# ponimatkin/freepose

Hardware: AMD Instinct MI355X
Metric: proposals/sec (ViT-L feat + top-k + 576-pose render-compare) (higher is better)
Workload: dtype bf16

## Files before the change

freepose_amd/_lib.py:

```python
from __future__ import annotations

import ctypes as C
import os
from pathlib import Path

_HERE = Path(__file__).resolve().parent
LIB_PATH = _HERE / "lib" / "libfreepose_hip.so"
LAB_LIB_PATH = _HERE / "lib" / "libfreepose_hip_lab.so"

_lib = None
_use_lab = False


def use_lab():
    global _use_lab
    if _lib is not None and not _use_lab:
        raise RuntimeError("use_lab() after the product library was loaded")
    _use_lab = True


def is_lab() -> bool:
    return _use_lab

c_void_p, c_int, c_float, c_double, c_size_t, c_char_p = C.c_void_p, C.c_int, C.c_float, C.c_double, C.c_size_t, C.c_char_p
# ... 4 lines not shown
    _fields_ = [("dim", c_int), ("depth", c_int), ("heads", c_int), ("mlp_dim", c_int), ("patch", c_int),
                ("n_reg", c_int), ("pos_grid", c_int), ("ln_eps", c_float)]


SIGNATURES = {
    "fp_last_error": (c_char_p, []),
    "fp_version": (c_int, []),
    "fp_ctx_create": (c_int, [c_int, P(c_void_p)]),
    "fp_ctx_destroy": (c_int, [c_void_p]),
    "fp_ctx_set_option": (c_int, [c_void_p, c_char_p, c_int]),
    "fp_ctx_workspace_bytes": (c_size_t, [c_void_p]),
    "fp_vit_create": (c_int, [c_void_p, P(VitArch), P(c_void_p)]),
    "fp_vit_destroy": (c_int, [c_void_p]),
    "fp_vit_set_weight": (c_int, [c_void_p, c_char_p, c_void_p, c_size_t, c_void_p]),
    "fp_vit_forward": (c_int, [c_void_p, c_void_p, c_int, c_int, c_int, c_int, c_int, c_void_p, c_void_p]),
    "fp_vit_flops": (c_double, [c_void_p, c_int, c_int, c_int, c_int]),
    "fp_ffa": (c_int, [c_void_p, c_void_p, c_void_p, c_int, c_int, c_int, c_int, c_int, c_int, c_void_p, c_void_p, c_void_p]),
    "fp_bank_prepare": (c_int, [c_void_p, c_void_p, c_int, c_int, c_void_p, c_void_p]),
    "fp_bank_topk": (c_int, [c_void_p, c_void_p, c_int, c_int, c_void_p, c_int, c_int, c_int, c_void_p, c_void_p, c_void_p]),
    "fp_topk_merge": (c_int, [c_void_p, c_void_p, c_void_p, c_int, c_int, c_int, c_void_p, c_void_p, c_void_p]),
    "fp_rerank_views": (c_int, [c_void_p, c_void_p, c_void_p, c_void_p, c_void_p, c_int, c_int, c_int, c_int, c_void_p, c_void_p]),
    "fp_l2_normalize": (c_int, [c_void_p, c_void_p, c_int, c_int, c_void_p, c_void_p]),
    "fp_template_score": (c_int, [c_void_p, c_void_p, c_void_p, c_void_p, c_int, c_int, c_int, c_void_p, c_void_p]),
    "fp_template_score_normed": (c_int, [c_void_p, c_void_p, c_void_p, c_void_p, c_int, c_int, c_int, c_void_p, c_void_p]),
    "fp_crop_resize_pad": (c_int, [c_void_p, c_void_p, c_int, c_int, c_int, c_int, c_int, c_void_p, c_int, c_float,
                                   c_int, c_void_p, c_int, c_void_p, c_int, c_void_p]),
    "fp_roi_align": (c_int, [c_void_p, c_void_p, c_int, c_int, c_int, c_int, c_void_p, c_int, c_int, c_int, c_int, c_float,
                             c_void_p, c_void_p]),
    "fp_generate_rotations": (c_int, [c_int, c_void_p]),
    "fp_geodesic_select": (c_int, [c_void_p, c_void_p, c_int, c_void_p, c_double, c_void_p, P(c_int), c_void_p]),
    "fp_mesh_upload": (c_int, [c_void_p, c_void_p, c_int, c_void_p, c_int, c_void_p, P(c_void_p)]),
    "fp_mesh_upload_textured": (c_int, [c_void_p, c_void_p, c_int, c_void_p, c_int, c_void_p, c_void_p, c_int, c_int, c_void_p,
                                        P(c_void_p)]),
    "fp_mesh_set_ambient": (c_int, [c_void_p, c_float]),
    "fp_mesh_set_shading": (c_int, [c_void_p, c_int]),
    "fp_mesh_set_filter": (c_int, [c_void_p, c_int]),
    "fp_mesh_set_cull": (c_int, [c_void_p, c_int]),
    "fp_project_vertices": (c_int, [c_void_p, c_void_p, c_void_p, c_int, c_float, c_float, c_float, c_float, c_float, c_void_p,
                                    c_void_p, c_void_p]),
    "fp_mesh_destroy": (c_int, [c_void_p]),
    "fp_rasterize": (c_int, [c_void_p, c_void_p, c_void_p, c_int, c_float, c_float, c_float, c_float, c_float, c_int,
# ... 81 lines not shown
```

freepose_amd/csrc/capi.hip:

```cpp
#include <stdarg.h>
#include <stdio.h>
#include <string.h>
#include <stdlib.h>

#include <cmath>

#include "../../include/freepose_hip.h"
#include "internal.h"

static thread_local char g_err[512] = "";
void fp_set_error(const char* fmt, ...) {
    va_list ap;
    va_start(ap, fmt);
    vsnprintf(g_err, sizeof(g_err), fmt, ap);
    va_end(ap);
}
extern "C" const char* fp_last_error(void) { return g_err; }
extern "C" int fp_version(void) { return 100; }

#ifdef FP_LAB
static int g_opts[FP_OPT_COUNT] = {-1, -1, -1, -1, -1, -1, -1, -1, -1, -1, -1, -1};
int fp_opt_get(int key, int dflt) { return (key >= 0 && key < FP_OPT_COUNT && g_opts[key] >= 0) ? g_opts[key] : dflt; }
extern "C" int fp_lab_set_option(const char* name, int value) {
    FP_REQUIRE(name, "lab_set_option: null name");
// ... 294 lines not shown
        if (v->ev_used == v->ev_pool.size()) {
            fp_vit::EvPair p{};
            if (hipEventCreate(&p.a) != hipSuccess || hipEventCreate(&p.b) != hipSuccess) return;
            v->ev_pool.push_back(p);
        }
        slot = v->ev_used++;
        v->ev_pool[slot].cls = cls;
        (void)hipEventRecord(v->ev_pool[slot].a, s);
    }
    ~ProfScope() {
        if (slot != (size_t)-1) (void)hipEventRecord(v->ev_pool[slot].b, s);
    }
};
}

extern "C" int fp_vit_forward(fp_vit* v, const void* d_images, int B, int H, int W, int layer, int feature_type,
                              void* d_out, void* stream) {
    FP_REQUIRE(v && d_images && d_out, "vit_forward: null argument");
    const fp_vit_arch& a = v->a;
    hipStream_t s = (hipStream_t)stream;
    FP_REQUIRE(B > 0 && H % a.patch == 0 && W % a.patch == 0, "vit_forward: B=%d H=%d W=%d (patch %d)", B, H, W, a.patch);
    FP_REQUIRE(feature_type >= 0 && feature_type <= 3, "vit_forward: feature_type %d", feature_type);
    FP_REQUIRE(v->cls && v->pos && v->pe_b && v->normw && v->normb && (a.n_reg == 0 || v->reg),
               "vit_forward: embedding / final-norm weights not set");
    const int L = (layer >= 1 && layer <= a.depth) ? layer : a.depth;
    for (int i = 0; i < L; ++i) {
        const VitBlockW& w = v->blk[i];
        FP_REQUIRE(w.n1w && w.n1b && w.qkvw && w.qkvb && w.projw && w.projb && w.n2w && w.n2b && w.fc1w && w.fc1b &&
                       w.fc2w && w.fc2b, "vit_forward: weights of block %d not set", i);
    }
    const int D = a.dim, gh = H / a.patch, gw = W / a.patch, P = gh * gw;
    const int n_tok = P + 1 + a.n_reg;
    const int npad = cdiv(n_tok, 16) * 16;
    const size_t M = (size_t)B * npad;
    FP_REQUIRE(M * (size_t)a.mlp_dim * 2 < 0xffffffffull, "vit_forward: batch too large for 32-bit tile offsets (B=%d)", B);

    bf16_t *A0, *X, *Y, *QK, *Vt, *AO, *H1;
    int rc;
    const int nosplit = v->ctx->opt_row_split == 0;
    const bool lnf = v->ctx->opt_ln_fused != 0 && D % 64 == 0;
    uint4* stat = nullptr;
    float2* part = nullptr;
    float* rstd = nullptr;
    if (lnf) {
        if (v->fold_ev && s != v->fold_stream) FP_HIP(hipStreamWaitEvent(s, v->fold_ev, 0));
        if (v->folded_upto < L) {
            if (v->refold) {
                FP_HIP(hipDeviceSynchronize());
                v->refold = false;
            }
            if ((rc = vit_fold(v, v->folded_upto, L, s))) return rc;
            if (!v->fold_ev) FP_HIP(hipEventCreateWithFlags(&v->fold_ev, hipEventDisableTiming));
            FP_HIP(hipEventRecord(v->fold_ev, s));
            v->fold_stream = s;
            v->folded_upto = L;
        }
        if ((rc = v->ctx->get("vit.ln_stat", M * sizeof(uint4), (void**)&stat))) return rc;
        if ((rc = v->ctx->get("vit.ln_rstd", M * sizeof(float), (void**)&rstd))) return rc;
        if ((rc = v->ctx->get("vit.ln_part", M * (size_t)(D / 64) * sizeof(float2), (void**)&part))) return rc;
    }
    if ((rc = v->ctx->get("vit.im2col", (size_t)B * P * v->KP * 2, (void**)&A0))) return rc;
    if ((rc = v->ctx->get("vit.x", M * D * 2, (void**)&X))) return rc;
    if ((rc = v->ctx->get("vit.y", M * D * 2, (void**)&Y))) return rc;
    if ((rc = v->ctx->get("vit.qk", M * 2 * D * 2, (void**)&QK))) return rc;
    if ((rc = v->ctx->get("vit.vt", M * D * 2 + 256, (void**)&Vt))) return rc;
    if ((rc = v->ctx->get("vit.ao", M * D * 2, (void**)&AO))) return rc;
    if ((rc = v->ctx->get("vit.h1", M * (size_t)a.mlp_dim * 2, (void**)&H1))) return rc;

    const bf16_t* pos_patch;
    if ((rc = vit_pos(v, gh, gw, s, &pos_patch))) return rc;

    {
        ProfScope ps(v, s, &v->ms_other);
        if ((rc = fp_im2col_norm((const bf16_t*)d_images, A0, B, H, W, a.patch, v->KP, s))) return rc;
        if ((rc = fp_token_init(X, v->cls, v->pos, v->reg, a.n_reg, B, n_tok, npad, D, s))) return rc;
    }
    {
        ProfScope ps(v, s, &v->ms_gemm);
        FpGemmArgs g{}; g.no_split = nosplit; if ((rc = v->ctx->sk_scratch(g, s))) return rc;
        g.X = A0; g.ldx = v->KP; g.W = v->pe_w; g.ldw = v->KP; g.C = X; g.ldc = D; g.bias = v->pe_b;
        g.M = B * P; g.N = D; g.K = v->KP; g.pos = pos_patch; g.P = P; g.npad = npad; g.tok_off = 1 + a.n_reg;
        if ((rc = fp_gemm_bf16(g, FP_EPI_PATCH, s))) return rc;
        if (v->prof) { v->gemm_flops += 2.0 * g.M * (3.0 * a.patch * a.patch) * D; v->gemm_launches += 1; }
    }
    const int Mi = (int)M;
    const double Malg = (double)B * n_tok;
    for (int i = 0; i < L; ++i) {
        const VitBlockW& w = v->blk[i];
        const fp_vit::VitFold& f = v->fold[i];
// ... 51 lines not shown
    }
    {
        ProfScope ps(v, s, &v->ms_other);
        int rows_per_b, off;
        if (feature_type == 0) { rows_per_b = 1; off = 0; }
        else if (feature_type == 1) { rows_per_b = a.n_reg; off = 1; }
        else { rows_per_b = P; off = 1 + a.n_reg; }
        if (rows_per_b > 0)
            if ((rc = fp_layernorm(X, (bf16_t*)d_out, v->normw, v->normb, B * rows_per_b, D, a.ln_eps, rows_per_b, npad,
                                   off, s, feature_type == 3)))
                return rc;
    }
    return FP_OK;
}

extern "C" int fp_vit_profile(fp_vit* v, int enable) {
    FP_REQUIRE(v, "vit_profile: null");
    v->prof = enable != 0;
    v->ev_used = 0;
    v->ms_gemm = v->ms_attn = v->ms_other = 0;
    v->gemm_flops = 0;
    v->gemm_launches = 0;
    return FP_OK;
}
extern "C" int fp_vit_profile_read(fp_vit* v, float* g, float* at, float* o, double* fl) {
    FP_REQUIRE(v, "vit_profile_read: null");
    float acc[3] = {0.f, 0.f, 0.f};
    for (size_t i = 0; i < v->ev_used; ++i) {
        FP_HIP(hipEventSynchronize(v->ev_pool[i].b));
        float ms = 0.f;
// ... 250 lines not shown
```

freepose_amd/csrc/internal.h:

```cpp
#pragma once
#include <algorithm>
#include <map>
#include <string>
#include <vector>

#include "common.h"
#include "gemm_bf16.h"

struct fp_ctx {
    int device = 0;
    struct Buf { void* p = nullptr; size_t bytes = 0; };
    std::map<std::string, Buf> bufs;
    int get(const char* name, size_t bytes, void** out);
    void* comm = nullptr;
    int comm_rank = 0, comm_size = 1;
    int opt_ln_fused = -1;
    int opt_raster_tiled = -1;
    int opt_comm_timeout_s = -1;
    int opt_row_split = -1;
    int opt_stream_k = -1;
    float* sk_ws = nullptr;
    int* sk_cnt = nullptr;
    static constexpr size_t SK_WS_BYTES = (size_t)64 << 20;
    static constexpr int SK_CNT_N = 16384;
    int sk_scratch(FpGemmArgs& g, hipStream_t s);
    int* ffa_arrive = nullptr;
    size_t total() const;
    void release();
};

constexpr float FP_ATTN_QSCALE = 1.4426950408889634f / 8.0f;
int fp_attention_fwd(const bf16_t* QK, int ldqk, const bf16_t* Vt, bf16_t* O, int ldo, int B, int H, int n_tok,
                     int npad, bool q_prescaled, hipStream_t stream);
int fp_im2col_norm(const bf16_t* img, bf16_t* A, int B, int H, int W, int ps, int KP, hipStream_t s);
int fp_token_init(bf16_t* X, const bf16_t* cls, const bf16_t* pos0, const bf16_t* reg, int nreg, int B, int n_tok,
                  int npad, int D, hipStream_t s);
int fp_layernorm(const bf16_t* X, bf16_t* Y, const bf16_t* gamma, const bf16_t* beta, int rows, int D, float eps,
                 int rows_per_b, int in_stride_b, int in_off, hipStream_t s, int l2_normalize = 0);
int fp_posembed_aa(const bf16_t* src, bf16_t* dst, int G, int gh, int gw, int D, hipStream_t s);
int fp_ffa_pool(const bf16_t* feats, const uint8_t* mask, bf16_t* out, float* out_f32, int B, int P, int D, int gh,
                int gw, int cell, uint8_t* pm_scratch, hipStream_t s, bf16_t* out_norm = nullptr, int* arrive = nullptr);
int fp_l2norm_rows(const bf16_t* X, bf16_t* Y, int rows, int D, hipStream_t s);
int fp_row_stats(const bf16_t* X, uint4* mfrag, float* rstd, int rows, int D, float eps, hipStream_t s);
int fp_stats_finalize(const float2* part, uint4* mfrag, float* rstd, int rows, int D, float eps, hipStream_t s, int part_ld = 0);
int fp_ln_fold(const bf16_t* W, const bf16_t* gamma, const bf16_t* beta, const bf16_t* bias, bf16_t* Wf, uint4* cfrag, int N, int K,
               int n_scaled, float row_scale, hipStream_t s);
int fp_cast_f32_bf16(const float* x, bf16_t* y, size_t n, hipStream_t s);
int fp_bank_scan(const bf16_t* bank, const bf16_t* queries, uint16_t* keys, int ldk, int N, int D, int Q, hipStream_t s);
// ... 17 lines not shown
```

freepose_amd/csrc/pose.hip:

```cpp
#include "internal.h"

namespace {

struct CropParam {
    int x0, y0, cw, ch;
    int h1, w1;
    int pad_t, pad_l;
    int S_h, S_w;
    float inv1, inv2;
    int out;
};

__global__ void crop_params_kernel(const int32_t* __restrict__ boxes, int n, int H, int W, float ext, int ext_is_zero,
                                   int target, CropParam* __restrict__ out) {
    const int i = blockIdx.x * blockDim.x + threadIdx.x;
    if (i >= n) return;
    int x0 = boxes[4 * i + 0], y0 = boxes[4 * i + 1], x1 = boxes[4 * i + 2], y1 = boxes[4 * i + 3];
    const int bw = x1 - x0, bh = y1 - y0;
    if (ext_is_zero) {
        x0 = max(0, x0); x1 = min(W, x1); y0 = max(0, y0); y1 = min(H, y1);
    } else {
        const float ew = ext * (float)bw, eh = ext * (float)bh;
        const float fx0 = (float)x0 - ew, fx1 = (float)x1 + ew, fy0 = (float)y0 - eh, fy1 = (float)y1 + eh;
        x0 = (fx0 > 0.f) ? (int)fx0 : 0;
// ... 168 lines not shown
                    if ((o & 3) == 0) *(uint2*)op = make_uint2(lo, hi);
                    else { ((uint32_t*)op)[0] = lo; ((uint32_t*)op)[1] = hi; }
                } else {
                    ((uint32_t*)op)[0] = lo;
                }
            } else {
                float* op = (float*)outp + o;
                if (nval == 4) {
                    if ((o & 3) == 0) *(float4*)op = make_float4(v[c][0], v[c][1], v[c][2], v[c][3]);
                    else { *(float2*)op = make_float2(v[c][0], v[c][1]); *(float2*)(op + 2) = make_float2(v[c][2], v[c][3]); }
                } else {
                    *(float2*)op = make_float2(v[c][0], v[c][1]);
                }
            }
        }
    }
}

struct Rot9 { double v[9]; };
__global__ void geodesic_flags_kernel(const double* __restrict__ grid, int G, const Rot9 Rprev,
                                      double thresh_deg, int32_t* __restrict__ flags) {
    const int i = blockIdx.x * blockDim.x + threadIdx.x;
    if (i >= G) return;
    const double* Rp = Rprev.v;
    double R[9], D[9];
    for (int k = 0; k < 9; ++k) R[k] = grid[(size_t)i * 9 + k];
    for (int r = 0; r < 3; ++r)
        for (int c = 0; c < 3; ++c) D[3 * r + c] = R[3 * r] * Rp[3 * c] + R[3 * r + 1] * Rp[3 * c + 1] + R[3 * r + 2] * Rp[3 * c + 2];
    const double cosv = 0.5 * (D[0] + D[4] + D[8] - 1.0);
    const double a = D[7] - D[5], b = D[2] - D[6], c = D[3] - D[1];
// ... 145 lines not shown
        if (src_u8 == 1) { if (out_bf16) FP_CROP_RGB(1, 1); else FP_CROP_RGB(1, 0); }
        else { if (out_bf16) FP_CROP_RGB(2, 1); else FP_CROP_RGB(2, 0); }
#undef FP_CROP_RGB
        FP_LAUNCH_CHECK();
        return FP_OK;
    }
#define FP_CROP(U, O) hipLaunchKernelGGL((crop_kernel<U, O>), grid, block, 0, s, images, n_img, C, H, W, params, target, masks, mask_mode, out)
    if (src_u8 == 1) { if (out_bf16) FP_CROP(1, 1); else FP_CROP(1, 0); }
    else if (src_u8 == 2) { if (out_bf16) FP_CROP(2, 1); else FP_CROP(2, 0); }
    else { if (out_bf16) FP_CROP(0, 1); else FP_CROP(0, 0); }
#undef FP_CROP
    FP_LAUNCH_CHECK();
    return FP_OK;
}

#include "../../include/freepose_hip.h"

extern "C" int fp_crop_resize_pad(fp_ctx* ctx, const void* d_images, int src_fmt, int n_img, int C, int H, int W,
                                  const int32_t* d_boxes, int n, float bbox_extend, int target, const uint8_t* d_masks,
                                  int mask_mode, void* d_out, int out_fmt, void* stream) {
    FP_REQUIRE(ctx && d_images && d_boxes && d_out, "crop_resize_pad: null argument");
    FP_REQUIRE(n_img == 1 || n_img == n, "crop_resize_pad: n_img must be 1 or n");
    FP_REQUIRE(mask_mode == 0 || d_masks, "crop_resize_pad: mask_mode %d needs masks", mask_mode);
    if (n == 0) return FP_OK;
    CropParam* params;
    int rc;
    if ((rc = ctx->get("crop.params", (size_t)n * sizeof(CropParam), (void**)&params))) return rc;
    return fp_crop_resize_pad_launch(d_images, src_fmt, n_img, C, H, W, d_boxes, n, bbox_extend, target, d_masks,
                                     mask_mode, d_out, out_fmt, params, (hipStream_t)stream);
}

extern "C" int fp_geodesic_select(fp_ctx* ctx, const double* d_grid, int G, const double* h_R, double thresh_deg,
                                  int32_t* d_out_idx, int* h_n, void* stream) {
    FP_REQUIRE(ctx && d_grid && h_R && d_out_idx && h_n, "geodesic_select: null argument");
    hipStream_t s = (hipStream_t)stream;
    char* ws;
    int rc;
    if ((rc = ctx->get("geo.ws", (size_t)G * 4 + 256, (void**)&ws))) return rc;
    int* dn = (int*)(ws + 128);
    int32_t* flags = (int32_t*)(ws + 256);
    Rot9 Rd;
    for (int i = 0; i < 9; ++i) Rd.v[i] = h_R[i];
    hipLaunchKernelGGL(geodesic_flags_kernel, dim3(cdiv(G, 256)), dim3(256), 0, s, d_grid, G, Rd, thresh_deg, flags);
    FP_LAUNCH_CHECK();
// ... 48 lines not shown
```

freepose_amd/csrc/vit_misc.hip:

```cpp
#include "internal.h"
#include "gemm_bf16.h"

namespace {

__global__ void im2col_norm_kernel(const bf16_t* __restrict__ img, bf16_t* __restrict__ A, int B, int H,
                                   int W, int ps, int KP, float m0, float m1, float m2, float s0, float s1,
                                   float s2) {
    const int gw = W / ps, gh = H / ps, P = gw * gh;
    const int K = 3 * ps * ps;
    const int chunks = KP / 8;
    const long total = (long)B * P * chunks;
    for (long idx = blockIdx.x * (long)blockDim.x + threadIdx.x; idx < total;
         idx += (long)gridDim.x * blockDim.x) {
        const int ch = (int)(idx % chunks);
        const long row = idx / chunks;
        const int b = (int)(row / P), pp = (int)(row % P);
        const int py = pp / gw, px = pp % gw;
        uint32_t w[4];
#pragma unroll
        for (int e = 0; e < 8; e += 2) {
            float v[2];
#pragma unroll
            for (int u = 0; u < 2; ++u) {
                const int k = ch * 8 + e + u;
                float val = 0.f;
                if (k < K) {
                    const int c = k / (ps * ps), rem = k % (ps * ps);
                    const int dy = rem / ps, dx = rem % ps;
                    const float x = bf2f(img[(((size_t)b * 3 + c) * H + (py * ps + dy)) * W + px * ps + dx]);
                    const float mean = c == 0 ? m0 : (c == 1 ? m1 : m2);
                    const float sd = c == 0 ? s0 : (c == 1 ? s1 : s2);
                    val = rbf(rbf(x - mean) / sd);
                }
                v[u] = val;
            }
            w[e / 2] = pack_bf2(v[0], v[1]);
        }
        *(uint4*)(A + (size_t)row * KP + ch * 8) = make_uint4(w[0], w[1], w[2], w[3]);
    }
}

__global__ void token_init_kernel(bf16_t* __restrict__ X, const bf16_t* __restrict__ cls,
                                  const bf16_t* __restrict__ pos0, const bf16_t* __restrict__ reg, int nreg,
                                  int n_tok, int npad, int D) {
    const int b = blockIdx.y;
    const int nrows = 1 + nreg + (npad - n_tok);
    for (int i = blockIdx.x * blockDim.x + threadIdx.x; i < nrows * D; i += gridDim.x * blockDim.x) {
        const int r = i / D, c = i % D;
        int row;
        bf16_t v;
        if (r == 0) { row = 0; v = f2bf(bf2f(cls[c]) + bf2f(pos0[c])); }
        else if (r <= nreg) { row = r; v = reg[(r - 1) * D + c]; }
        else { row = n_tok + (r - 1 - nreg); v = 0; }
// ... 388 lines not shown
    hipLaunchKernelGGL(stats_finalize_kernel, dim3(cdiv(rows, 256)), dim3(256), 0, s, part, ms, rstd, rows, D / 64, 1.0f / (float)D, eps, part_ld > 0 ? part_ld : rows);
    FP_LAUNCH_CHECK();
    return FP_OK;
}

int fp_ln_fold(const bf16_t* W, const bf16_t* gamma, const bf16_t* beta, const bf16_t* bias, bf16_t* Wf, uint4* cb, int N, int K,
               int n_scaled, float row_scale, hipStream_t s) {
    FP_REQUIRE(W && gamma && beta && bias && Wf && cb, "ln_fold: null argument (W / LayerNorm gamma, beta / bias / outputs)");
    FP_REQUIRE(N > 0 && K % 8 == 0, "ln_fold: N=%d, K=%d (K must be a multiple of 8)", N, K);
    hipLaunchKernelGGL(ln_fold_kernel, dim3(cdiv(N, 4)), dim3(256), 0, s, W, gamma, beta, bias, Wf, cb, N, K, n_scaled, row_scale);
    FP_LAUNCH_CHECK();
    return FP_OK;
}

int fp_im2col_norm(const bf16_t* img, bf16_t* A, int B, int H, int W, int ps, int KP, hipStream_t s) {
    FP_REQUIRE(H % ps == 0 && W % ps == 0 && KP % 8 == 0 && KP >= 3 * ps * ps, "im2col: bad shape");
    const long total = (long)B * (H / ps) * (W / ps) * (KP / 8);
    const int blocks = (int)std::min<long>((total + 255) / 256, 256 * 16);
    hipLaunchKernelGGL(im2col_norm_kernel, dim3(blocks), dim3(256), 0, s, img, A, B, H, W, ps, KP, rbf(0.485f),
                       rbf(0.456f), rbf(0.406f), rbf(0.229f), rbf(0.224f), rbf(0.225f));
    FP_LAUNCH_CHECK();
    return FP_OK;
}

int fp_token_init(bf16_t* X, const bf16_t* cls, const bf16_t* pos0, const bf16_t* reg, int nreg, int B,
                  int n_tok, int npad, int D, hipStream_t s) {
    const int nrows = 1 + nreg + (npad - n_tok);
    hipLaunchKernelGGL(token_init_kernel, dim3(cdiv(nrows * D, 256), B), dim3(256), 0, s, X, cls, pos0, reg, nreg,
                       n_tok, npad, D);
    FP_LAUNCH_CHECK();
    return FP_OK;
}

int fp_layernorm(const bf16_t* X, bf16_t* Y, const bf16_t* gamma, const bf16_t* beta, int rows, int D, float eps,
                 int rows_per_b, int in_stride_b, int in_off, hipStream_t s, int l2_normalize) {
// ... 52 lines not shown
```

freepose_amd/ops.py:

```python
from __future__ import annotations

import ctypes as C
import functools
from typing import Optional

import numpy as np
import torch

from . import _lib
from ._lib import check, current_stream, ptr

_ctx = {}


def context(device: Optional[int] = None):
    if device is None:
        device = torch.cuda.current_device()
    h = _ctx.get(device)
    if h is None:
        lib = _lib.load()
        out = C.c_void_p()
        check(lib.fp_ctx_create(int(device), C.byref(out)), "fp_ctx_create")
        h = _ctx[device] = out
    return h
# ... 62 lines not shown
        B, Cc, H, W = x.shape
        assert Cc == 3
        P = (H // self.patch) * (W // self.patch)
        ft = FEATURE_TYPES[feature_type]
        shape = {0: (B, self.dim), 1: (B, self.n_reg, self.dim), 2: (B, P, self.dim), 3: (B, P, self.dim)}[ft]
        if out is None:
            out = torch.empty(shape, dtype=torch.bfloat16, device=x.device)
        else:
            assert tuple(out.shape) == shape and out.dtype == torch.bfloat16 and out.is_contiguous() and out.device == x.device
        if B > 0:
            check(self.lib.fp_vit_forward(self.handle, ptr(x), B, H, W, int(layer), ft, ptr(out), current_stream()),
                  "fp_vit_forward")
        return out

    __call__ = forward

    def flops(self, B, H, W, layer=22) -> float:
        return float(self.lib.fp_vit_flops(self.handle, B, H, W, layer))

    def profile(self, enable: bool):
        check(self.lib.fp_vit_profile(self.handle, int(enable)))

    def profile_read(self):
        g, a, o, f = C.c_float(), C.c_float(), C.c_float(), C.c_double()
        check(self.lib.fp_vit_profile_read(self.handle, C.byref(g), C.byref(a), C.byref(o), C.byref(f)))
        return {"ms_gemm": g.value, "ms_attn": a.value, "ms_other": o.value, "gemm_flops": f.value,
                "gemm_launches": int(self.lib.fp_vit_profile_gemm_launches(self.handle))}

    def __del__(self):
        try:
# ... 144 lines not shown
        img = _dev(images, torch.float32)
        n_img, Cc, H, W = img.shape
        src = 0
    bx = _dev(boxes).to(torch.int32).contiguous()
    n = bx.shape[0]
    m = _dev(masks).to(torch.uint8).contiguous() if masks is not None else None
    if mask_mode == 2:
        Cc_out = 1
    else:
        Cc_out = Cc
    out = torch.empty((n, Cc_out, target, target), dtype=torch.bfloat16 if out_bf16 else torch.float32, device=img.device)
    if n:
        check(lib.fp_crop_resize_pad(context(), ptr(img), src, n_img, Cc_out if mask_mode == 2 else Cc, H, W, ptr(bx), n,
                                     float(bbox_extend), int(target), ptr(m), int(mask_mode), ptr(out), int(out_bf16),
                                     current_stream()), "fp_crop_resize_pad")
    return out


def roi_align(images: torch.Tensor, rois: torch.Tensor, output_size, sampling_ratio: int = 2,
              spatial_scale: float = 1.0) -> torch.Tensor:
    lib = _lib.load()
    img = _dev(images, torch.float32)
    r = _dev(rois, torch.float32).reshape(-1, 5).contiguous()
    ph, pw = (output_size, output_size) if isinstance(output_size, int) else output_size
    N, Cc, H, W = img.shape
    n = r.shape[0]
    out = torch.empty((n, Cc, ph, pw), dtype=torch.float32, device=img.device)
    if n:
        check(lib.fp_roi_align(context(), ptr(img), N, Cc, H, W, ptr(r), n, int(ph), int(pw), int(sampling_ratio),
                               float(spatial_scale), ptr(out), current_stream()), "fp_roi_align")
# ... 392 lines not shown
```

freepose_amd/pipeline.py:

```python
from __future__ import annotations

from dataclasses import dataclass
from typing import List, Optional

import numpy as np
import torch

from freepose_amd import ops, parallel
from freepose_amd.retrieval import TemplateBank
from freepose_amd.src.pipeline.retrieval.renderer import MeshRenderer, grid_poses
from freepose_amd.src.pipeline.utils import z_from_extents


class StageClock:

    def __init__(self):
        self._spans = []
        self._pool = []

    class _Span:
        def __init__(self, clock, name):
            self.clock, self.name = clock, name

        def __enter__(self):
# ... 49 lines not shown
        self._poses_dev = torch.from_numpy(self.hyp_poses.astype(np.float32)).cuda()
        self.fx = self.fy = 600.0 * render_res / 420.0
        self.cx = self.cy = render_res / 2
        self.clock = _NoClock()

    def retrieve(self, crops: torch.Tensor, masks: torch.Tensor):
        with self.clock.stage("vit_query"):
            feats = self.vit(crops, layer=self.layer, feature_type="patch")
        g = self.crop_res // 14
        with self.clock.stage("ffa"):
            desc = ops.ffa(feats, masks[:, : g * 14, : g * 14], cell=14, normalize=True)
        with self.clock.stage("bank_scan_topk"):
            s, i = self.bank.topk(desc, self.k)
        return feats, s, i

    def render_hypotheses(self):
        with self.clock.stage("rasterize"):
            rgb, _, ext, boxes = ops.rasterize_extents(self.mesh, self._poses_dev, self.render_scale, self.fx, self.fy, self.cx, self.cy,
                                                       self.render_res, self.render_res)
        with self.clock.stage("crop_resize"):
            crops = ops.crop_resize_pad(rgb, boxes, self.crop_res, 0.0, out_bf16=True)
        return crops, ext

    def hypothesis_features(self, crops: torch.Tensor, normalized: bool = False) -> torch.Tensor:
        g = self.crop_res // 14
        sizes = ops.plan_vit_batches(crops.shape[0], g * g + 5, self.vit_batch)
        with self.clock.stage("vit_hypotheses"):
            feats = torch.empty((crops.shape[0], g * g, self.vit.dim), dtype=torch.bfloat16, device=crops.device)
            i = 0
            for b in sizes:
                self.vit(crops[i:i + b], layer=self.layer, feature_type="patch_normalized" if normalized else "patch", out=feats[i:i + b])
                i += b
            return feats

    def run(self, crops: torch.Tensor, masks: torch.Tensor, K: np.ndarray, bboxes: np.ndarray, scales) -> List[ProposalResult]:
        feats, top_s, top_i = self.retrieve(crops, masks)
        out = []
        for b in range(crops.shape[0]):
            hyp_crops, ext = self.render_hypotheses()
            hyp_feats = self.hypothesis_features(hyp_crops, normalized=True)
            with self.clock.stage("template_score"):
                q = ops.l2_normalize(feats[b])
                scores = ops.template_score(hyp_feats, q, normalized=True)
            with self.clock.stage("hypothesis_top3"):
                idx_all = torch.arange(self.n_hyp, dtype=torch.int32, device=scores.device)
                s3, i3 = ops.topk_merge(scores[None], idx_all[None], 3)
            k = top_s.shape[1]
            packed = torch.cat([i3[0].double(), s3[0].double(), ext[i3[0].long(), 4:6].double().reshape(-1), top_s[b].double(),
                                top_i[b].double()]).cpu().numpy()
            i3h = packed[0:3].astype(np.int64)
            s3h = packed[3:6].astype(np.float32)
            e = packed[6:12].reshape(3, 2)
            ratio = float(scales[b]) / self.render_scale
            tco = [z_from_extents(bboxes[b], e[j, 0] * ratio, e[j, 1] * ratio, K, self.hyp_poses[i3h[j]]) for j in range(3)]
# ... 9 lines not shown
```

include/freepose_hip.h:

```cpp
#ifndef FREEPOSE_HIP_H
#define FREEPOSE_HIP_H
#include <stddef.h>
#include <stdint.h>

#ifdef __cplusplus
extern "C" {
#endif

#define FP_OK 0
#define FP_ERR_INVALID 1
#define FP_ERR_HIP 2
#define FP_ERR_STATE 3

typedef struct fp_ctx fp_ctx;
typedef struct fp_vit fp_vit;
typedef struct fp_mesh fp_mesh;

const char* fp_last_error(void);
int fp_version(void);
int fp_ctx_create(int device, fp_ctx** out);
int fp_ctx_destroy(fp_ctx* ctx);
int fp_ctx_set_option(fp_ctx* ctx, const char* name, int value);
size_t fp_ctx_workspace_bytes(const fp_ctx* ctx);

// ... 1 lines not shown
    int dim;
    int depth;
    int heads;
    int mlp_dim;
    int patch;
    int n_reg;
    int pos_grid;
    float ln_eps;
} fp_vit_arch;

int fp_vit_create(fp_ctx* ctx, const fp_vit_arch* arch, fp_vit** out);
int fp_vit_destroy(fp_vit* vit);
int fp_vit_set_weight(fp_vit* vit, const char* name, const void* d_bf16, size_t numel, void* stream);
int fp_vit_forward(fp_vit* vit, const void* d_images, int B, int H, int W, int layer, int feature_type,
                   void* d_out_bf16, void* stream);
double fp_vit_flops(const fp_vit* vit, int B, int H, int W, int layer);

int fp_ffa(fp_ctx* ctx, const void* d_feats, const uint8_t* d_mask, int B, int gh, int gw, int D, int cell,
           int normalize, void* d_out_bf16, float* d_out_f32, void* stream);

int fp_bank_prepare(fp_ctx* ctx, const float* d_bank_f32, int N, int D, void* d_bank_bf16, void* stream);
int fp_bank_topk(fp_ctx* ctx, const void* d_bank_bf16, int N, int D, const void* d_queries, int Q, int k,
                 int idx_offset, float* d_out_scores, int32_t* d_out_idx, void* stream);
int fp_topk_merge(fp_ctx* ctx, const float* d_cand_scores, const int32_t* d_cand_idx, int Q, int C, int k,
                  float* d_out_scores, int32_t* d_out_idx, void* stream);
int fp_rerank_views(fp_ctx* ctx, const void* d_views, const int32_t* d_offsets, const int32_t* d_cand,
                    const void* d_queries, int Q, int C, int D, int k, float* d_out, void* stream);
int fp_l2_normalize(fp_ctx* ctx, const void* d_x_bf16, int rows, int D, void* d_y_bf16, void* stream);

int fp_template_score(fp_ctx* ctx, const void* d_tmpl, const void* d_query, const float* d_weights, int T, int P,
                      int D, float* d_scores, void* stream);
int fp_template_score_normed(fp_ctx* ctx, const void* d_tmpl_normed, const void* d_query, const float* d_weights, int T,
                             int P, int D, float* d_scores, void* stream);

int fp_crop_resize_pad(fp_ctx* ctx, const void* d_images, int src_fmt, int n_img, int C, int H, int W,
                       const int32_t* d_boxes, int n, float bbox_extend, int target, const uint8_t* d_masks,
                       int mask_mode, void* d_out, int out_fmt, void* stream);

int fp_roi_align(fp_ctx* ctx, const float* d_images, int n_img, int C, int H, int W, const float* d_rois, int n,
                 int pooled_h, int pooled_w, int sampling_ratio, float spatial_scale, float* d_out, void* stream);

int fp_generate_rotations(int n, double* h_out);
int fp_geodesic_select(fp_ctx* ctx, const double* d_grid, int G, const double* h_Rprev9, double thresh_deg,
                       int32_t* d_out_idx, int* h_n, void* stream);

int fp_mesh_upload(fp_ctx* ctx, const float* h_verts, int V, const int32_t* h_faces, int F,
                   const uint8_t* h_colors, fp_mesh** out);
int fp_mesh_upload_textured(fp_ctx* ctx, const float* h_verts, int V, const int32_t* h_faces, int F, const float* h_uv,
                            const uint8_t* h_texture, int th, int tw, const float* h_kd3, fp_mesh** out);
int fp_mesh_destroy(fp_mesh* mesh);
int fp_mesh_set_ambient(fp_mesh* mesh, float ambient);
int fp_mesh_set_shading(fp_mesh* mesh, int mode);
// ... 57 lines not shown
```

Baseline: 2.035.

## Fuse hypothesis crop-resize with im2col normalization into ViT patch rows

Adds a crop kernel that writes normalized bf16 patch rows directly in the ViT's im2col layout, plus a ViT entry point that consumes those rows. This skips the intermediate crop image and the separate im2col pass for the 576 rendered hypotheses. The generic im2col kernel is also reorganized into per-patch-row blocks with paired loads. The cost is a second code path whose bf16 rounding has to match the existing crop-then-normalize path exactly.

```diff
diff --git a/freepose_amd/_lib.py b/freepose_amd/_lib.py
--- a/freepose_amd/_lib.py
+++ b/freepose_amd/_lib.py
@@ -42,6 +42,8 @@
     "fp_vit_destroy": (c_int, [c_void_p]),
     "fp_vit_set_weight": (c_int, [c_void_p, c_char_p, c_void_p, c_size_t, c_void_p]),
     "fp_vit_forward": (c_int, [c_void_p, c_void_p, c_int, c_int, c_int, c_int, c_int, c_void_p, c_void_p]),
+    "fp_vit_forward_patches": (c_int, [c_void_p, c_void_p, c_int, c_int, c_int, c_int, c_int, c_void_p, c_void_p]),
+    "fp_vit_patch_kp": (c_int, [c_void_p]),
     "fp_vit_flops": (c_double, [c_void_p, c_int, c_int, c_int, c_int]),
     "fp_ffa": (c_int, [c_void_p, c_void_p, c_void_p, c_int, c_int, c_int, c_int, c_int, c_int, c_void_p, c_void_p, c_void_p]),
     "fp_bank_prepare": (c_int, [c_void_p, c_void_p, c_int, c_int, c_void_p, c_void_p]),
@@ -53,6 +55,8 @@
     "fp_template_score_normed": (c_int, [c_void_p, c_void_p, c_void_p, c_void_p, c_int, c_int, c_int, c_void_p, c_void_p]),
     "fp_crop_resize_pad": (c_int, [c_void_p, c_void_p, c_int, c_int, c_int, c_int, c_int, c_void_p, c_int, c_float,
                                    c_int, c_void_p, c_int, c_void_p, c_int, c_void_p]),
+    "fp_crop_resize_patches": (c_int, [c_void_p, c_void_p, c_int, c_int, c_int, c_int, c_int, c_void_p, c_int, c_float,
+                                       c_int, c_void_p, c_int, c_int, c_int, c_void_p, c_void_p]),
     "fp_roi_align": (c_int, [c_void_p, c_void_p, c_int, c_int, c_int, c_int, c_void_p, c_int, c_int, c_int, c_int, c_float,
                              c_void_p, c_void_p]),
     "fp_generate_rotations": (c_int, [c_int, c_void_p]),
diff --git a/freepose_amd/csrc/capi.hip b/freepose_amd/csrc/capi.hip
--- a/freepose_amd/csrc/capi.hip
+++ b/freepose_amd/csrc/capi.hip
@@ -332,9 +332,9 @@
 };
 }
 
-extern "C" int fp_vit_forward(fp_vit* v, const void* d_images, int B, int H, int W, int layer, int feature_type,
-                              void* d_out, void* stream) {
-    FP_REQUIRE(v && d_images && d_out, "vit_forward: null argument");
+static int vit_forward_body(fp_vit* v, const void* d_images, const void* d_patches, int B, int H, int W, int layer, int feature_type,
+                            void* d_out, void* stream) {
+    FP_REQUIRE(v && (d_images || d_patches) && d_out, "vit_forward: null argument");
     const fp_vit_arch& a = v->a;
     hipStream_t s = (hipStream_t)stream;
     FP_REQUIRE(B > 0 && H % a.patch == 0 && W % a.patch == 0, "vit_forward: B=%d H=%d W=%d (patch %d)", B, H, W, a.patch);
@@ -353,7 +353,8 @@
     const size_t M = (size_t)B * npad;
     FP_REQUIRE(M * (size_t)a.mlp_dim * 2 < 0xffffffffull, "vit_forward: batch too large for 32-bit tile offsets (B=%d)", B);
 
-    bf16_t *A0, *X, *Y, *QK, *Vt, *AO, *H1;
+    const bf16_t* A0 = (const bf16_t*)d_patches;
+    bf16_t *X, *Y, *QK, *Vt, *AO, *H1;
     int rc;
     const int nosplit = v->ctx->opt_row_split == 0;
     const bool lnf = v->ctx->opt_ln_fused != 0 && D % 64 == 0;
@@ -377,7 +378,11 @@
         if ((rc = v->ctx->get("vit.ln_rstd", M * sizeof(float), (void**)&rstd))) return rc;
         if ((rc = v->ctx->get("vit.ln_part", M * (size_t)(D / 64) * sizeof(float2), (void**)&part))) return rc;
     }
-    if ((rc = v->ctx->get("vit.im2col", (size_t)B * P * v->KP * 2, (void**)&A0))) return rc;
+    bf16_t* A0w = nullptr;
+    if (!d_patches) {
+        if ((rc = v->ctx->get("vit.im2col", (size_t)B * P * v->KP * 2, (void**)&A0w))) return rc;
+        A0 = A0w;
+    }
     if ((rc = v->ctx->get("vit.x", M * D * 2, (void**)&X))) return rc;
     if ((rc = v->ctx->get("vit.y", M * D * 2, (void**)&Y))) return rc;
     if ((rc = v->ctx->get("vit.qk", M * 2 * D * 2, (void**)&QK))) return rc;
@@ -390,7 +395,7 @@
 
     {
         ProfScope ps(v, s, &v->ms_other);
-        if ((rc = fp_im2col_norm((const bf16_t*)d_images, A0, B, H, W, a.patch, v->KP, s))) return rc;
+        if (!d_patches && (rc = fp_im2col_norm((const bf16_t*)d_images, A0w, B, H, W, a.patch, v->KP, s))) return rc;
         if ((rc = fp_token_init(X, v->cls, v->pos, v->reg, a.n_reg, B, n_tok, npad, D, s))) return rc;
     }
     {
@@ -472,6 +477,20 @@
     return FP_OK;
 }
 
+extern "C" int fp_vit_forward(fp_vit* v, const void* d_images, int B, int H, int W, int layer, int feature_type,
+                              void* d_out, void* stream) {
+    FP_REQUIRE(d_images, "vit_forward: null argument");
+    return vit_forward_body(v, d_images, nullptr, B, H, W, layer, feature_type, d_out, stream);
+}
+
+extern "C" int fp_vit_forward_patches(fp_vit* v, const void* d_patches, int B, int H, int W, int layer, int feature_type,
+                                      void* d_out, void* stream) {
+    FP_REQUIRE(d_patches && ((uintptr_t)d_patches & 15) == 0, "vit_forward_patches: null or unaligned patch rows");
+    return vit_forward_body(v, nullptr, d_patches, B, H, W, layer, feature_type, d_out, stream);
+}
+
+extern "C" int fp_vit_patch_kp(const fp_vit* v) { return v ? v->KP : 0; }
+
 extern "C" int fp_vit_profile(fp_vit* v, int enable) {
     FP_REQUIRE(v, "vit_profile: null");
     v->prof = enable != 0;
diff --git a/freepose_amd/csrc/internal.h b/freepose_amd/csrc/internal.h
--- a/freepose_amd/csrc/internal.h
+++ b/freepose_amd/csrc/internal.h
@@ -32,6 +32,13 @@
 constexpr float FP_ATTN_QSCALE = 1.4426950408889634f / 8.0f;
 int fp_attention_fwd(const bf16_t* QK, int ldqk, const bf16_t* Vt, bf16_t* O, int ldo, int B, int H, int n_tok,
                      int npad, bool q_prescaled, hipStream_t stream);
+struct FpImgNorm { float m0, m1, m2, s0, s1, s2; };
+static inline FpImgNorm fp_imagenet_norm() { return {rbf(0.485f), rbf(0.456f), rbf(0.406f), rbf(0.229f), rbf(0.224f), rbf(0.225f)}; }
+__device__ __forceinline__ float fp_patch_norm(float x, int c, const FpImgNorm& n) {
+    const float mean = c == 0 ? n.m0 : (c == 1 ? n.m1 : n.m2);
+    const float sd = c == 0 ? n.s0 : (c == 1 ? n.s1 : n.s2);
+    return rbf(rbf(x - mean) / sd);
+}
 int fp_im2col_norm(const bf16_t* img, bf16_t* A, int B, int H, int W, int ps, int KP, hipStream_t s);
 int fp_token_init(bf16_t* X, const bf16_t* cls, const bf16_t* pos0, const bf16_t* reg, int nreg, int B, int n_tok,
                   int npad, int D, hipStream_t s);
diff --git a/freepose_amd/csrc/pose.hip b/freepose_amd/csrc/pose.hip
--- a/freepose_amd/csrc/pose.hip
+++ b/freepose_amd/csrc/pose.hip
@@ -206,6 +206,80 @@
                 }
             }
         }
+    }
+}
+
+constexpr int CROP_PS_MAX = 32;
+template <int SRC_U8, int PS>
+__global__ __launch_bounds__(256) void crop_patches_kernel(const void* __restrict__ images, int n_img, int H, int W,
+                                                           const CropParam* __restrict__ params, int target, int ps_rt,
+                                                           const uint8_t* __restrict__ masks, int mask_mode,
+                                                           bf16_t* __restrict__ A, int KP, FpImgNorm nm) {
+    __shared__ unsigned short ntab[3][257];
+    __shared__ short xs_s[2048];
+    __shared__ int ys_s[CROP_PS_MAX];
+    const int ps = PS ? PS : ps_rt, pp = ps * ps;
+    const int t = threadIdx.x;
+    if (SRC_U8 != 0) {
+        const float v = rbf((SRC_U8 == 1) ? (float)((double)t / 255.0) : __fdiv_rn((float)t, 255.0f));
+#pragma unroll
+        for (int c = 0; c < 3; ++c) {
+            ntab[c][t] = f2bf(fp_patch_norm(v, c, nm));
+            if (t == 0) ntab[c][256] = f2bf(fp_patch_norm(0.f, c, nm));
+        }
+    }
+    const int i = blockIdx.y, py = blockIdx.x;
+    const CropParam p = params[i];
+    const int img = (n_img == 1) ? 0 : i;
+    const bool geom = (p.out == target) && p.cw > 0 && p.ch > 0;
+    const bool small1 = (p.h1 + p.w1) <= 128, small2 = (2 * p.out) <= 128;
+    for (int ox = t; ox < target; ox += blockDim.x) {
+        int xs = -1;
+        if (geom) {
+            const int x1 = nearest_src(ox, p.S_w, p.out, p.inv2, small2) - p.pad_l;
+            if (x1 >= 0 && x1 < p.w1) xs = p.x0 + nearest_src(x1, p.cw, p.w1, p.inv1, small1);
+        }
+        xs_s[ox] = (short)xs;
+    }
+    if (t < ps) {
+        int ys = -1;
+        if (geom) {
+            const int y1 = nearest_src(py * ps + t, p.S_h, p.out, p.inv2, small2) - p.pad_t;
+            if (y1 >= 0 && y1 < p.h1) ys = p.y0 + nearest_src(y1, p.ch, p.h1, p.inv1, small1);
+        }
+        ys_s[t] = ys;
+    }
+    __syncthreads();
+    const int gw = target / ps, chunks = KP / 8;
+    bf16_t* dst = A + ((size_t)i * gw * gw + (size_t)py * gw) * KP;
+    const bool masked = masks && mask_mode != 0;
+    for (int item = t; item < gw * chunks; item += blockDim.x) {
+        const int px = item / chunks, ch = item - px * chunks;
+        const int k0 = ch * 8;
+        int c = k0 / pp, dy = (k0 - c * pp) / ps, dx = k0 - c * pp - dy * ps;
+        uint32_t bits[8];
+#pragma unroll
+        for (int e = 0; e < 8; ++e) {
+            bits[e] = 0;
+            if (c < 3) {
+                const int ys = ys_s[dy], xs = xs_s[px * ps + dx];
+                const bool ok = ys >= 0 && xs >= 0;
+                float m = 1.f;
+                if (ok && masked) m = masks[((size_t)i * H + ys) * W + xs] ? 1.f : 0.f;
+                if (SRC_U8 != 0) {
+                    int idx = 256;
+                    if (ok && m != 0.f) idx = ((const uint8_t*)images)[(((size_t)img * H + ys) * W + xs) * 3 + c];
+                    bits[e] = ntab[c][idx];
+                } else {
+                    float v = 0.f;
+                    if (ok) v = ((const float*)images)[(((size_t)img * 3 + c) * H + ys) * W + xs] * m;
+                    bits[e] = f2bf(fp_patch_norm(rbf(v), c, nm));
+                }
+                if (++dx == ps) { dx = 0; if (++dy == ps) { dy = 0; ++c; } }
+            }
+        }
+        *(uint4*)(dst + (size_t)px * KP + k0) = make_uint4(bits[0] | (bits[1] << 16), bits[2] | (bits[3] << 16), bits[4] | (bits[5] << 16),
+                                                           bits[6] | (bits[7] << 16));
     }
 }
 
@@ -381,6 +455,22 @@
     return FP_OK;
 }
 
+int fp_crop_resize_patches_launch(const void* images, int src_u8, int n_img, int H, int W, const int32_t* boxes, int n,
+                                  float bbox_extend, int target, const uint8_t* masks, int mask_mode, int ps, int KP, bf16_t* A,
+                                  CropParam* params, hipStream_t s) {
+    hipLaunchKernelGGL(crop_params_kernel, dim3(cdiv(n, 64)), dim3(64), 0, s, boxes, n, H, W, bbox_extend,
+                       bbox_extend == 0.f ? 1 : 0, target, params);
+    FP_LAUNCH_CHECK();
+    const dim3 grid(target / ps, n), block(256);
+    const FpImgNorm nm = fp_imagenet_norm();
+#define FP_CROP_PATCHES(U, P) hipLaunchKernelGGL((crop_patches_kernel<U, P>), grid, block, 0, s, images, n_img, H, W, params, target, ps, masks, mask_mode, A, KP, nm)
+    if (ps == 14) { if (src_u8 == 1) FP_CROP_PATCHES(1, 14); else if (src_u8 == 2) FP_CROP_PATCHES(2, 14); else FP_CROP_PATCHES(0, 14); }
+    else { if (src_u8 == 1) FP_CROP_PATCHES(1, 0); else if (src_u8 == 2) FP_CROP_PATCHES(2, 0); else FP_CROP_PATCHES(0, 0); }
+#undef FP_CROP_PATCHES
+    FP_LAUNCH_CHECK();
+    return FP_OK;
+}
+
 #include "../../include/freepose_hip.h"
 
 extern "C" int fp_crop_resize_pad(fp_ctx* ctx, const void* d_images, int src_fmt, int n_img, int C, int H, int W,
@@ -395,6 +485,25 @@
     if ((rc = ctx->get("crop.params", (size_t)n * sizeof(CropParam), (void**)&params))) return rc;
     return fp_crop_resize_pad_launch(d_images, src_fmt, n_img, C, H, W, d_boxes, n, bbox_extend, target, d_masks,
                                      mask_mode, d_out, out_fmt, params, (hipStream_t)stream);
+}
+
+extern "C" int fp_crop_resize_patches(fp_ctx* ctx, const void* d_images, int src_fmt, int n_img, int C, int H, int W,
+                                      const int32_t* d_boxes, int n, float bbox_extend, int target, const uint8_t* d_masks,
+                                      int mask_mode, int patch, int KP, void* d_A, void* stream) {
+    FP_REQUIRE(ctx && d_images && d_boxes && d_A, "crop_resize_patches: null argument");
+    FP_REQUIRE(n_img == 1 || n_img == n, "crop_resize_patches: n_img must be 1 or n");
+    FP_REQUIRE(src_fmt >= 0 && src_fmt <= 2 && C == 3, "crop_resize_patches: src_fmt %d, C=%d (the ViT takes 3 channels)", src_fmt, C);
+    FP_REQUIRE(mask_mode == 0 || (mask_mode == 1 && d_masks), "crop_resize_patches: mask_mode %d (0, or 1 with masks)", mask_mode);
+    FP_REQUIRE(patch > 0 && patch <= CROP_PS_MAX && target > 0 && target % patch == 0 && target <= 2048 && W <= 32767,
+               "crop_resize_patches: target=%d patch=%d W=%d unsupported", target, patch, W);
+    FP_REQUIRE(KP % 8 == 0 && KP >= 3 * patch * patch && ((uintptr_t)d_A & 15) == 0, "crop_resize_patches: KP=%d / unaligned output", KP);
+    FP_REQUIRE(n <= 65535, "crop_resize_patches: %d boxes are too many for one launch", n);
+    if (n <= 0) return FP_OK;
+    CropParam* params;
+    int rc;
+    if ((rc = ctx->get("crop.params", (size_t)n * sizeof(CropParam), (void**)&params))) return rc;
+    return fp_crop_resize_patches_launch(d_images, src_fmt, n_img, H, W, d_boxes, n, bbox_extend, target, d_masks, mask_mode, patch,
+                                         KP, (bf16_t*)d_A, params, (hipStream_t)stream);
 }
 
 extern "C" int fp_geodesic_select(fp_ctx* ctx, const double* d_grid, int G, const double* h_R, double thresh_deg,
diff --git a/freepose_amd/csrc/vit_misc.hip b/freepose_amd/csrc/vit_misc.hip
--- a/freepose_amd/csrc/vit_misc.hip
+++ b/freepose_amd/csrc/vit_misc.hip
@@ -3,40 +3,46 @@
 
 namespace {
 
-__global__ void im2col_norm_kernel(const bf16_t* __restrict__ img, bf16_t* __restrict__ A, int B, int H,
-                                   int W, int ps, int KP, float m0, float m1, float m2, float s0, float s1,
-                                   float s2) {
-    const int gw = W / ps, gh = H / ps, P = gw * gh;
-    const int K = 3 * ps * ps;
+template <int PS, int PAIR>
+__global__ __launch_bounds__(256) void im2col_norm_kernel(const bf16_t* __restrict__ img, bf16_t* __restrict__ A, int H, int W,
+                                                          int ps_rt, int KP, int npx, int segs, FpImgNorm nm) {
+    const int ps = PS ? PS : ps_rt, pp = ps * ps;
+    const int gw = W / ps, gh = H / ps;
+    const int py = blockIdx.x / segs, px0 = (blockIdx.x - py * segs) * npx, b = blockIdx.y;
+    const int n = min(npx, gw - px0);
     const int chunks = KP / 8;
-    const long total = (long)B * P * chunks;
-    for (long idx = blockIdx.x * (long)blockDim.x + threadIdx.x; idx < total;
-         idx += (long)gridDim.x * blockDim.x) {
-        const int ch = (int)(idx % chunks);
-        const long row = idx / chunks;
-        const int b = (int)(row / P), pp = (int)(row % P);
-        const int py = pp / gw, px = pp % gw;
+    const bf16_t* src = img + ((size_t)b * 3 * H + (size_t)py * ps) * W;
+    bf16_t* dst = A + ((size_t)b * gh * gw + (size_t)py * gw + px0) * KP;
+    for (int item = threadIdx.x; item < n * chunks; item += blockDim.x) {
+        const int p = item / chunks, ch = item - p * chunks;
+        const int k0 = ch * 8;
+        int c = k0 / pp, dy = (k0 - c * pp) / ps, dx = k0 - c * pp - dy * ps;
+        const int x0 = (px0 + p) * ps;
         uint32_t w[4];
 #pragma unroll
-        for (int e = 0; e < 8; e += 2) {
-            float v[2];
-#pragma unroll
-            for (int u = 0; u < 2; ++u) {
-                const int k = ch * 8 + e + u;
-                float val = 0.f;
-                if (k < K) {
-                    const int c = k / (ps * ps), rem = k % (ps * ps);
-                    const int dy = rem / ps, dx = rem % ps;
-                    const float x = bf2f(img[(((size_t)b * 3 + c) * H + (py * ps + dy)) * W + px * ps + dx]);
-                    const float mean = c == 0 ? m0 : (c == 1 ? m1 : m2);
-                    const float sd = c == 0 ? s0 : (c == 1 ? s1 : s2);
-                    val = rbf(rbf(x - mean) / sd);
-                }
-                v[u] = val;
-            }
-            w[e / 2] = pack_bf2(v[0], v[1]);
-        }
-        *(uint4*)(A + (size_t)row * KP + ch * 8) = make_uint4(w[0], w[1], w[2], w[3]);
+        for (int e = 0; e < 4; ++e) {
+            float v0 = 0.f, v1 = 0.f;
+            if (PAIR) {
+                if (c < 3) {
+                    const uint32_t q = *(const uint32_t*)(src + ((size_t)c * H + dy) * W + x0 + dx);
+                    v0 = fp_patch_norm(lo_bf(q), c, nm);
+                    v1 = fp_patch_norm(hi_bf(q), c, nm);
+                    dx += 2;
+                    if (dx == ps) { dx = 0; if (++dy == ps) { dy = 0; ++c; } }
+                }
+            } else {
+                if (c < 3) {
+                    v0 = fp_patch_norm(bf2f(src[((size_t)c * H + dy) * W + x0 + dx]), c, nm);
+                    if (++dx == ps) { dx = 0; if (++dy == ps) { dy = 0; ++c; } }
+                }
+                if (c < 3) {
+                    v1 = fp_patch_norm(bf2f(src[((size_t)c * H + dy) * W + x0 + dx]), c, nm);
+                    if (++dx == ps) { dx = 0; if (++dy == ps) { dy = 0; ++c; } }
+                }
+            }
+            w[e] = pack_bf2(v0, v1);
+        }
+        *(uint4*)(dst + (size_t)p * KP + k0) = make_uint4(w[0], w[1], w[2], w[3]);
     }
 }
 
@@ -455,11 +461,18 @@
 }
 
 int fp_im2col_norm(const bf16_t* img, bf16_t* A, int B, int H, int W, int ps, int KP, hipStream_t s) {
-    FP_REQUIRE(H % ps == 0 && W % ps == 0 && KP % 8 == 0 && KP >= 3 * ps * ps, "im2col: bad shape");
-    const long total = (long)B * (H / ps) * (W / ps) * (KP / 8);
-    const int blocks = (int)std::min<long>((total + 255) / 256, 256 * 16);
-    hipLaunchKernelGGL(im2col_norm_kernel, dim3(blocks), dim3(256), 0, s, img, A, B, H, W, ps, KP, rbf(0.485f),
-                       rbf(0.456f), rbf(0.406f), rbf(0.229f), rbf(0.224f), rbf(0.225f));
+    FP_REQUIRE(ps > 0 && H % ps == 0 && W % ps == 0 && KP % 8 == 0 && KP >= 3 * ps * ps, "im2col: bad shape");
+    FP_REQUIRE(B <= 65535, "im2col: batch %d too large for one launch", B);
+    if (B <= 0 || H == 0 || W == 0) return FP_OK;
+    const int gh = H / ps, gw = W / ps;
+    const int segs0 = std::max(1, std::min(cdiv(gw, 3), 2048 / std::max(1, gh * B)));
+    const int npx = cdiv(gw, segs0), segs = cdiv(gw, npx);
+    const bool pair = (W & 1) == 0 && (ps & 1) == 0 && ((uintptr_t)img & 3) == 0;
+    const FpImgNorm nm = fp_imagenet_norm();
+    const dim3 grid(gh * segs, B), block(256);
+    if (pair && ps == 14) hipLaunchKernelGGL((im2col_norm_kernel<14, 1>), grid, block, 0, s, img, A, H, W, ps, KP, npx, segs, nm);
+    else if (pair) hipLaunchKernelGGL((im2col_norm_kernel<0, 1>), grid, block, 0, s, img, A, H, W, ps, KP, npx, segs, nm);
+    else hipLaunchKernelGGL((im2col_norm_kernel<0, 0>), grid, block, 0, s, img, A, H, W, ps, KP, npx, segs, nm);
     FP_LAUNCH_CHECK();
     return FP_OK;
 }
diff --git a/freepose_amd/ops.py b/freepose_amd/ops.py
--- a/freepose_amd/ops.py
+++ b/freepose_amd/ops.py
@@ -100,6 +100,27 @@
         return out
 
     __call__ = forward
+
+    @property
+    def patch_kp(self) -> int:
+        return int(self.lib.fp_vit_patch_kp(self.handle))
+
+    def forward_patches(self, patches: torch.Tensor, H: int, W: int, layer: int = 22, feature_type: str = "cls",
+                        out: Optional[torch.Tensor] = None) -> torch.Tensor:
+        P = (H // self.patch) * (W // self.patch)
+        assert patches.is_cuda and patches.dtype == torch.bfloat16 and patches.is_contiguous() and patches.dim() == 2
+        assert patches.shape[1] == self.patch_kp and patches.shape[0] % P == 0, (tuple(patches.shape), P, self.patch_kp)
+        B = patches.shape[0] // P
+        ft = FEATURE_TYPES[feature_type]
+        shape = {0: (B, self.dim), 1: (B, self.n_reg, self.dim), 2: (B, P, self.dim), 3: (B, P, self.dim)}[ft]
+        if out is None:
+            out = torch.empty(shape, dtype=torch.bfloat16, device=patches.device)
+        else:
+            assert tuple(out.shape) == shape and out.dtype == torch.bfloat16 and out.is_contiguous() and out.device == patches.device
+        if B > 0:
+            check(self.lib.fp_vit_forward_patches(self.handle, ptr(patches), B, H, W, int(layer), ft, ptr(out), current_stream()),
+                  "fp_vit_forward_patches")
+        return out
 
     def flops(self, B, H, W, layer=22) -> float:
         return float(self.lib.fp_vit_flops(self.handle, B, H, W, layer))
@@ -274,6 +295,29 @@
         check(lib.fp_crop_resize_pad(context(), ptr(img), src, n_img, Cc_out if mask_mode == 2 else Cc, H, W, ptr(bx), n,
                                      float(bbox_extend), int(target), ptr(m), int(mask_mode), ptr(out), int(out_bf16),
                                      current_stream()), "fp_crop_resize_pad")
+    return out
+
+
+def crop_resize_patches(images: torch.Tensor, boxes: torch.Tensor, target: int, bbox_extend: float = 0.0,
+                        masks: Optional[torch.Tensor] = None, mask_mode: int = 0, u8_float_div: bool = False, ps: int = 14,
+                        kp: Optional[int] = None) -> torch.Tensor:
+    lib = _lib.load()
+    if images.dtype == torch.uint8:
+        img = _dev(images)
+        n_img, H, W, Cc = img.shape
+        src = 2 if u8_float_div else 1
+    else:
+        img = _dev(images, torch.float32)
+        n_img, Cc, H, W = img.shape
+        src = 0
+    bx = _dev(boxes).to(torch.int32).contiguous()
+    n = bx.shape[0]
+    m = _dev(masks).to(torch.uint8).contiguous() if masks is not None else None
+    kp = kp or (3 * ps * ps + 63) // 64 * 64
+    out = torch.empty((n * (target // ps) ** 2, kp), dtype=torch.bfloat16, device=img.device)
+    if n:
+        check(lib.fp_crop_resize_patches(context(), ptr(img), src, n_img, Cc, H, W, ptr(bx), n, float(bbox_extend), int(target), ptr(m),
+                                         int(mask_mode), int(ps), int(kp), ptr(out), current_stream()), "fp_crop_resize_patches")
     return out
 
 
diff --git a/freepose_amd/pipeline.py b/freepose_amd/pipeline.py
--- a/freepose_amd/pipeline.py
+++ b/freepose_amd/pipeline.py
@@ -87,22 +87,31 @@
             s, i = self.bank.topk(desc, self.k)
         return feats, s, i
 
-    def render_hypotheses(self):
+    def render_hypotheses(self, patch_rows: bool = False):
         with self.clock.stage("rasterize"):
             rgb, _, ext, boxes = ops.rasterize_extents(self.mesh, self._poses_dev, self.render_scale, self.fx, self.fy, self.cx, self.cy,
                                                        self.render_res, self.render_res)
         with self.clock.stage("crop_resize"):
-            crops = ops.crop_resize_pad(rgb, boxes, self.crop_res, 0.0, out_bf16=True)
+            if patch_rows:
+                crops = ops.crop_resize_patches(rgb, boxes, self.crop_res, 0.0, ps=self.vit.patch, kp=self.vit.patch_kp)
+            else:
+                crops = ops.crop_resize_pad(rgb, boxes, self.crop_res, 0.0, out_bf16=True)
         return crops, ext
 
     def hypothesis_features(self, crops: torch.Tensor, normalized: bool = False) -> torch.Tensor:
         g = self.crop_res // 14
-        sizes = ops.plan_vit_batches(crops.shape[0], g * g + 5, self.vit_batch)
+        rows = crops.dim() == 2
+        n = crops.shape[0] // (g * g) if rows else crops.shape[0]
+        sizes = ops.plan_vit_batches(n, g * g + 5, self.vit_batch)
+        ft = "patch_normalized" if normalized else "patch"
         with self.clock.stage("vit_hypotheses"):
-            feats = torch.empty((crops.shape[0], g * g, self.vit.dim), dtype=torch.bfloat16, device=crops.device)
+            feats = torch.empty((n, g * g, self.vit.dim), dtype=torch.bfloat16, device=crops.device)
             i = 0
             for b in sizes:
-                self.vit(crops[i:i + b], layer=self.layer, feature_type="patch_normalized" if normalized else "patch", out=feats[i:i + b])
+                if rows:
+                    self.vit.forward_patches(crops[i * g * g:(i + b) * g * g], g * 14, g * 14, layer=self.layer, feature_type=ft, out=feats[i:i + b])
+                else:
+                    self.vit(crops[i:i + b], layer=self.layer, feature_type=ft, out=feats[i:i + b])
                 i += b
             return feats
 
@@ -110,7 +119,7 @@
         feats, top_s, top_i = self.retrieve(crops, masks)
         out = []
         for b in range(crops.shape[0]):
-            hyp_crops, ext = self.render_hypotheses()
+            hyp_crops, ext = self.render_hypotheses(patch_rows=True)
             hyp_feats = self.hypothesis_features(hyp_crops, normalized=True)
             with self.clock.stage("template_score"):
                 q = ops.l2_normalize(feats[b])
diff --git a/include/freepose_hip.h b/include/freepose_hip.h
--- a/include/freepose_hip.h
+++ b/include/freepose_hip.h
@@ -39,6 +39,9 @@
 int fp_vit_set_weight(fp_vit* vit, const char* name, const void* d_bf16, size_t numel, void* stream);
 int fp_vit_forward(fp_vit* vit, const void* d_images, int B, int H, int W, int layer, int feature_type,
                    void* d_out_bf16, void* stream);
+int fp_vit_forward_patches(fp_vit* vit, const void* d_patches, int B, int H, int W, int layer, int feature_type,
+                           void* d_out_bf16, void* stream);
+int fp_vit_patch_kp(const fp_vit* vit);
 double fp_vit_flops(const fp_vit* vit, int B, int H, int W, int layer);
 
 int fp_ffa(fp_ctx* ctx, const void* d_feats, const uint8_t* d_mask, int B, int gh, int gw, int D, int cell,
@@ -61,6 +64,10 @@
 int fp_crop_resize_pad(fp_ctx* ctx, const void* d_images, int src_fmt, int n_img, int C, int H, int W,
                        const int32_t* d_boxes, int n, float bbox_extend, int target, const uint8_t* d_masks,
                        int mask_mode, void* d_out, int out_fmt, void* stream);
+
+int fp_crop_resize_patches(fp_ctx* ctx, const void* d_images, int src_fmt, int n_img, int C, int H, int W,
+                           const int32_t* d_boxes, int n, float bbox_extend, int target, const uint8_t* d_masks,
+                           int mask_mode, int patch, int KP, void* d_A, void* stream);
 
 int fp_roi_align(fp_ctx* ctx, const float* d_images, int n_img, int C, int H, int W, const float* d_rois, int n,
                  int pooled_h, int pooled_w, int sampling_ratio, float spatial_scale, float* d_out, void* stream);
```

New measurement: 2.040 (median of 6 runs). About the same (+0.2%).
